# kcroker/Gadget-2.0.7-ngravs

Hardware: AMD Instinct MI355X
Metric: particle-steps/s (tree+PM) (higher is better)
Workload: dtype f64

## Files before the change

gadget-2.0.7-ngravs_amd/csrc/capi.hip:

```cpp
#include "engine.hpp"
#include "../../include/ngravs_peano.h"
#include <chrono>
#include <cmath>

static thread_local std::string g_create_error;

void ngravs_report(ngravs_ctx *ctx, int code, const std::string &msg)
{
  if(ctx)
    ctx->last_error = msg;
  else
    g_create_error = msg;
  if(ctx && ctx->on_fatal)
    ctx->on_fatal(code, msg.c_str());
  else
    fprintf(stderr, "task %d: endrun called with an error level of %d (%s)\n", ctx ? ctx->cfg.rank : 0, code, msg.c_str());
}

__global__ void k_pack_strided_f64(const unsigned char *src, long long stride, int ncomp, long long n, double *dst)
{
  long long i = blockIdx.x * (long long)blockDim.x + threadIdx.x;
  if(i >= n)
    return;
  const double *s = reinterpret_cast<const double *>(src + i * stride);
// ... 942 lines not shown
      return NGRAVS_ERR_NO_DEVICE;
    }
  uint32_t gp[8] = {0}, gw[8] = {0};
  if(hipExtStreamGetCUMask(sp, 8, gp) != hipSuccess || hipExtStreamGetCUMask(sw, 8, gw) != hipSuccess || memcmp(gp, mp, sizeof mp) ||
     memcmp(gw, mw, sizeof mw))
    {
      (void)hipStreamDestroy(sp);
      (void)hipStreamDestroy(sw);
      (void)hipGetLastError();
      return NGRAVS_ERR_NO_DEVICE;
    }
  c->pm_stream = sp;
  c->walk_stream = sw;
  c->pm_stream_cus = R;
  return NGRAVS_OK;
}

static bool overlap_eligible(const ngravs_ctx *c)
{
  return c->cfg.pmgrid && c->cfg.periodic && c->cfg.world_size == 1 && !c->top.on && c->cfg.walk_mode == NGRAVS_WALK_GROUP &&
         c->n > 0 && c->n_local > 0;
}

static int gravity_tree_impl(ngravs_ctx *c, hipEvent_t pm_done)
{
  if(!c || !c->have_order)
    return NGRAVS_ERR_STATE;
  (void)hipSetDevice(c->cfg.device);
  int rc;
  if(!c->have_tree)
    {
      int64_t nn = ngravs_force_treebuild(c);
      if(nn < 0)
        return (int)nn;
    }
  else if(c->tree_stale && (rc = ngravs_force_update_tree(c)))
    return rc;
  if((rc = ensure_table(c)))
    return rc;
  if(c->n_local == 0)
    {
      c->stats.t_treewalk = 0;
      c->stats.walk_kernel_ms = 0;
      c->stats.interactions = 0;
      c->stats.n_active = 0;
      c->have_acc = true;
      return NGRAVS_OK;
    }
  HIP_TRY(c, hipEventRecord(c->ev0, c->stream));
  const bool masked = (pm_done || (c->tune.pm_cus > 0 && overlap_eligible(c))) && masked_streams(c, pm_done ? c->pm_stream_cus : c->tune.pm_cus) == NGRAVS_OK;
  if(masked)
    {
      HIP_TRY(c, hipStreamWaitEvent(c->walk_stream, c->ev0, 0));
      {
        OnStream on(c, c->walk_stream, c->device_cus - c->pm_stream_cus);
        if((rc = walk_run(c)))
          return rc;
      }
      HIP_TRY(c, hipEventRecord(c->ev_walk, c->walk_stream));
      HIP_TRY(c, hipStreamWaitEvent(c->stream, c->ev_walk, 0));
    }
  else if((rc = walk_run(c)))
    return rc;
  if(pm_done)
    HIP_TRY(c, hipStreamWaitEvent(c->stream, pm_done, 0));
  if((rc = walk_finish(c)))
    return rc;
  HIP_TRY(c, hipEventRecord(c->ev1, c->stream));
  c->stats.t_treewalk = ev_ms(c) * 1e-3;
  float kms = 0;
  (void)hipEventSynchronize(c->evk1);
  (void)hipEventElapsedTime(&kms, c->evk0, c->evk1);
  c->stats.walk_kernel_ms = kms;
  double h[2] = {0, 0};
  HIP_TRY(c, hipMemcpyAsync(h, c->red_tmp.p, 2 * sizeof(double), hipMemcpyDeviceToHost, c->stream));
  HIP_TRY(c, hipStreamSynchronize(c->stream));
  c->stats.interactions = h[0];
  c->stats.n_active = (int64_t)h[1];
  c->have_acc = true;
  if(c->cfg.pmgrid && c->cfg.walk_mode == NGRAVS_WALK_GROUP && h[1] > 0 && c->cfg.box_size > 0)
    {
      const double reach = (c->cfg.group_reach > 0 ? c->cfg.group_reach : NGRAVS_GROUP_REACH) * c->asmth;
      const double ntot = c->top.on && c->top.total_count > 0 ? c->top.total_count : (double)c->n;
      const double L = c->cfg.box_size, expect = 4.18879020478639 * reach * reach * reach * ntot / (L * L * L);
      const bool dense = c->walk_ntargets < 0 || c->walk_dense_tlist;
      if(expect > 0 && dense)
        {
          const double f_sg = c->walk_sg >= 4 ? 1.0 : (c->walk_sg >= 2 ? 1857.0 / 1393.0 : 1857.0 / 1079.0);
          const double f_s = c->walk_spread >= 2 ? 1079.0 / 871.0 : 1.0;
          c->walk_ia_ratio = (h[0] / h[1]) / expect * f_sg * f_s;
        }
    }
  if(c->shard_count > 0 && c->extent_override)
    hipLaunchKernelGGL(k_cost_update, GRID1(c->shard_count), 0, c->stream, c->s_idx.p, c->s_active.p, c->r_nint.p,
                       (long long)c->shard_first, (long long)c->shard_count, c->in_cost.p);
  return NGRAVS_OK;
}

extern "C" int ngravs_gravity_tree(ngravs_ctx *c) { return gravity_tree_impl(c, nullptr); }

static int pm_on_masked_stream(ngravs_ctx *c)
{
  HIP_TRY(c, hipEventRecord(c->ev_fork, c->stream));
  HIP_TRY(c, hipStreamWaitEvent(c->pm_stream, c->ev_fork, 0));
  OnStream on(c, c->pm_stream, c->pm_stream_cus);
  HIP_TRY(c, hipEventRecord(c->ev_pm0, c->stream));
  int rc = pm_run(c);
  if(rc)
    return rc;
  HIP_TRY(c, hipEventRecord(c->ev_pm1, c->stream));
  return NGRAVS_OK;
}

extern "C" int ngravs_pmforce_periodic(ngravs_ctx *c)
{
  if(!c || !c->have_particles)
    return NGRAVS_ERR_STATE;
  (void)hipSetDevice(c->cfg.device);
  int rc;
  if(!c->have_order && (rc = ngravs_domain_decomposition(c)))
    return rc;
  if(!c->have_tree)
// ... 45 lines not shown
            c->pm_auto_cus = 8 * m;
          break;
        }
    }
  return c->pm_auto_cus;
}

extern "C" int ngravs_compute_accelerations(ngravs_ctx *c, int pm_step)
{
  if(!c || !c->have_particles)
    return NGRAVS_ERR_STATE;
  int rc;
  if((rc = domain_decomposition_impl(c, !(pm_step && c->cfg.pmgrid))))
    return rc;
  c->last_pm_cus = 0;
  if(!(pm_step && c->cfg.pmgrid))
    return ngravs_gravity_tree(c);
  const int R = choose_pm_cus(c);
  if(R > 0 && masked_streams(c, R) == NGRAVS_OK)
    {
      int64_t nn = ngravs_force_treebuild(c);
      if(nn < 0)
        return (int)nn;
      if((rc = pm_on_masked_stream(c)))
        return rc;
      if((rc = gravity_tree_impl(c, c->ev_pm1)))
        return rc;
      float ms = 0;
      (void)hipEventElapsedTime(&ms, c->ev_pm0, c->ev_pm1);
      c->stats.t_pm = ms * 1e-3;
      c->last_pm_cus = R;
      if(c->tune.pm_cus < 0 && ms > c->stats.walk_kernel_ms)
        c->pm_auto_cus = R < 32 ? R + 8 : 0;
      return NGRAVS_OK;
    }
  if((rc = ngravs_pmforce_periodic(c)))
    return rc;
  if((rc = ngravs_gravity_tree(c)))
    return rc;
  if(overlap_eligible(c) && c->tune.pm_cus < 0 && c->pm_auto_cus < 0)
    {
      c->pm_solo_ms = c->stats.t_pm * 1e3;
      c->walk_solo_ms = c->stats.walk_kernel_ms;
      c->pm_solo_steps++;
    }
  return NGRAVS_OK;
}

static int download_strided(ngravs_ctx *c, const void *dsrc, size_t elem, int ncomp, int64_t n, void *dst, int64_t stride,
// ... 1035 lines not shown
```

gadget-2.0.7-ngravs_amd/csrc/engine.hpp:

```cpp
#pragma once
#include <hip/hip_runtime.h>
#include <cstdint>
#include <cstdio>
#include <cstdlib>
#include <cstring>
#include <string>
#include <vector>
#include "../../include/ngravs_host.h"

#define NG_MAX NGRAVS_MAX_GRAVS
#define NTAB NGRAVS_NTAB
#define TREE_BITS NGRAVS_TREE_BITS
#define FLAG_BUCKET 64
#define FLAG_PSEUDO 128
#define FLAG_PARTIAL 256
#define MAX_LEVELS (TREE_BITS + 1)

struct ngravs_ctx;

#define HIP_TRY(ctx, expr)                                                                        \
  do                                                                                              \
    {                                                                                             \
      hipError_t e__ = (expr);                                                                    \
      if(e__ != hipSuccess)                                                                       \
        {                                                                                         \
          ngravs_report(ctx, NGRAVS_ERR_NO_DEVICE, std::string(#expr) + ": " + hipGetErrorString(e__)); \
          return NGRAVS_ERR_NO_DEVICE;                                                            \
        }                                                                                         \
    }                                                                                             \
  while(0)

void ngravs_report(ngravs_ctx *ctx, int code, const std::string &msg);

template <typename T> struct DevBuf
{
  T *p = nullptr;
  size_t cap = 0;
  int ensure(size_t n)
// ... 231 lines not shown
  long long walk_unopened = 0;
  int walk_unit_state = 4;
  double walk_ia_ratio = 0;
  bool all_active = true;
  DevBuf<int> walk_ovf;
  DevBuf<int> walk_counters;
  DevBuf<double> r_acc, r_pm, r_oldacc;
  DevBuf<int> r_nint;
  int pm_plan_n = 0;
  void *fft_fwd = nullptr, *fft_inv = nullptr;
  DevBuf<double> pm_rho;
  DevBuf<double> pm_force;
  DevBuf<double> pm_phi;
  DevBuf<double> pm_orig;
  DevBuf<double> out_tmp;
  DevBuf<float> out_tmpf;
  std::vector<unsigned char> host_stage;
  ngravs_stats_t stats;
  hipEvent_t ev0 = nullptr, ev1 = nullptr, evk0 = nullptr, evk1 = nullptr;
  std::vector<hipEvent_t> ev_batch;
  int walk_batches = 0;
  int walk_lcap = 0;
  int walk_scap = 0;
  std::string last_error;
  std::vector<ngravs_user_fn_t> user_fns;
  std::vector<ngravs_user_lattice_t> user_lat;
  DevBuf<double> user_tab;
  UserTabs user_ut = {};
  bool user_ready = false;
  double user_soft[NGRAVS_NTYPES] = {0, 0, 0, 0, 0, 0};
  int last_walk_kernel = 0;
  hipStream_t pm_stream = nullptr, walk_stream = nullptr;
  int pm_stream_cus = 0;
  int device_cus = 0;
  int stream_cus = 0;
  int last_pm_cus = 0;
  double pm_solo_ms = 0, walk_solo_ms = 0;
  int pm_solo_steps = 0;
  int pm_auto_cus = -1;
  hipEvent_t ev_fork = nullptr, ev_pm0 = nullptr, ev_pm1 = nullptr, ev_walk = nullptr;
  DevBuf<int> probe_out;
  DevBuf<double> user_green;
  long long user_green_nk2 = 0;
  DevBuf<double> sph_vel_in, sph_h_in;
  DevBuf<double> sph_vel;
  DevBuf<int> sph_tlist;
// ... 64 lines not shown
         (cfg.law_spline[i][j] >= NGRAVS_SPLINE_BAMBAM && cfg.law_spline[i][j] < NGRAVS_SPLINE_USER0))
        return true;
  return false;
}
static inline bool cfg_has_user(const ngravs_config_t &cfg)
{
  for(int i = 0; i < cfg.n_gravs; i++)
    for(int j = 0; j < cfg.n_gravs; j++)
      if(cfg.law_accel[i][j] >= NGRAVS_LAW_USER0 || cfg.law_spline[i][j] >= NGRAVS_SPLINE_USER0)
        return true;
  return false;
}
int user_check_config(const ngravs_config_t *cfg, const ngravs_user_fn_t *fns, int nfns, const ngravs_user_lattice_t *lat, int nlat,
                      std::string &why);
ngravs_lattice_fn user_lattice_fn(const ngravs_ctx *c, int a, int b);
bool user_lattice_complete(const ngravs_ctx *c);
int user_lattice_tabulate(ngravs_lattice_fn fn, double box, double *out, std::string &why);
void ngravs_report(ngravs_ctx *ctx, int code, const std::string &msg);
int user_tables_ensure(ngravs_ctx *c, double r_need);
int user_green_ensure(ngravs_ctx *c);
double user_normed(const ngravs_user_fn_t *fns, int nfns, int law, double k2);
void make_walk_params(const ngravs_ctx *c, WalkParams *wp);
int walk_run(ngravs_ctx *c);
int walk_finish(ngravs_ctx *c);
int direct_run(ngravs_ctx *c, const int *d_idx, int64_t nt, double *d_acc);
int direct_run_targets(ngravs_ctx *c, const double4 *d_tpm, const int *d_ttype, int64_t nt, double *d_acc, double r_need = 0);
int eval_ring_slots(const WalkParams &wp, bool yuk, int waves);
int launch_eval_ring(ngravs_ctx *c, const TreeView &tv, const WalkParams &wp, bool yuk, int nblk, int waves, int K, const int *region,
                     const int *gcount, long long g0, long long nb, int lcap, int scap, int S, const int *tlist, int SG, long long t_count);
#define SPH_KC1 2.546479089470
#define SPH_KC2 15.278874536822
#define SPH_KC3 45.836623610466
#define SPH_KC4 30.557749073644
#define SPH_KC5 5.092958178941
#define SPH_KC6 (-15.278874536822)
#define SPH_NORM_COEFF 4.188790204786
#define SPH_MAXITER 150
__host__ __device__ inline void sph_spline(double u, double hinv3, double hinv4, double *wk, double *dwk)
{
  if(u < 0.5)
    {
      *wk = hinv3 * (SPH_KC1 + SPH_KC2 * (u - 1) * u * u);
      *dwk = hinv4 * u * (SPH_KC3 * u - SPH_KC4);
    }
  else
    {
// ... 53 lines not shown
```

gadget-2.0.7-ngravs_amd/csrc/kernels_tree.hip:

```cpp
#include "engine.hpp"
#include <hipcub/hipcub.hpp>


__device__ __forceinline__ int key_digit(unsigned long long k, int level)
{
  return (int)((k >> (3 * (TREE_BITS - 1 - level))) & 7ull);
}

#define TB 128

__global__ __launch_bounds__(TB) void k_split(const unsigned long long *__restrict__ key, const int *__restrict__ n_first,
                                              const int *__restrict__ n_count, const int *__restrict__ lv, int level,
                                              int *__restrict__ n_child, int *__restrict__ n_nchild, int *__restrict__ blocksum,
                                              const int *__restrict__ n_top = nullptr, const int *__restrict__ t_child = nullptr,
                                              const int *__restrict__ t_gcnt = nullptr)
{
  __shared__ int wsum[TB / 64];
  const int node0 = lv[2 * level], nnodes_level = lv[2 * level + 1];
  const int nvb = (nnodes_level + TB - 1) / TB;
  for(int vb = blockIdx.x; vb < nvb; vb += gridDim.x)
    {
      const int t = vb * TB + threadIdx.x;
      int nn = 0;
      if(t < nnodes_level)
// ... 464 lines not shown
                          const int *__restrict__ n_first, const int *__restrict__ n_count,
                          const int *__restrict__ n_child, const double4 *__restrict__ n_geo,
                          double4 *__restrict__ n_mom, int *__restrict__ n_flags, int node0, int nnodes_level,
                          WalkParams wp, double4 *__restrict__ geo_rw = nullptr, int *__restrict__ n_npart = nullptr,
                          int *__restrict__ n_count_rw = nullptr)
{
  int t = blockIdx.x * blockDim.x + threadIdx.x;
  if(t >= nnodes_level)
    return;
  int node = node0 + t;
  double m[NG], sx[NG], sy[NG], sz[NG];
  int np[NG];
#pragma unroll
  for(int g = 0; g < NG; g++)
    {
      m[g] = sx[g] = sy[g] = sz[g] = 0;
      np[g] = 0;
    }
  SoftAcc sa;
  sa.maxsofttype = 7;
  sa.diff = 0;
  int cnt_acc = 0;
  int fl = n_flags[node];
  const double4 geo0 = n_geo[node];
  double need = 0;
  auto add_particle_v = [&](const double4 v, const int ty) {
    if(geo_rw)
      need = fmax(need, fmax(fabs(v.x - geo0.x), fmax(fabs(v.y - geo0.y), fabs(v.z - geo0.z))));
    int gg = wp.t2g[ty];
#pragma unroll
    for(int g = 0; g < NG; g++)
      if(g == gg)
        {
          np[g]++;
          m[g] += v.w;
          sx[g] += v.w * v.x;
          sy[g] += v.w * v.y;
          sz[g] += v.w * v.z;
        }
    soft_merge(sa, ty, 0, wp.fsoft);
    cnt_acc++;
  };
  auto add_particle = [&](int p) {
    double4 v = s_pm[p];
    if(geo_rw)
      need = fmax(need, fmax(fabs(v.x - geo0.x), fmax(fabs(v.y - geo0.y), fabs(v.z - geo0.z))));
    int ty = s_type[p];
    int gg = wp.t2g[ty];
#pragma unroll
    for(int g = 0; g < NG; g++)
      if(g == gg)
        {
          np[g]++;
          m[g] += v.w;
          sx[g] += v.w * v.x;
          sy[g] += v.w * v.y;
          sz[g] += v.w * v.z;
        }
    soft_merge(sa, ty, 0, wp.fsoft);
    cnt_acc++;
  };
  if(fl & FLAG_BUCKET)
    {
      int f = n_first[node], cnt = n_count[node];
      for(int p = f; p < f + cnt; p++)
        add_particle(p);
    }
  else
    {
      const int4 *cp = reinterpret_cast<const int4 *>(n_child + 8 * (long long)node);
      const int4 c_lo = cp[0], c_hi = cp[1];
      const int ch[8] = {c_lo.x, c_lo.y, c_lo.z, c_lo.w, c_hi.x, c_hi.y, c_hi.z, c_hi.w};
      constexpr int B = NG == 1 ? 4 : 2;
#pragma unroll
      for(int k0 = 0; k0 < 8; k0 += B)
        {
          double4 rec[B][NG];
          int aux[B], cnt_c[B];
#pragma unroll
          for(int q = 0; q < B; q++)
            {
              const int c = ch[k0 + q];
              aux[q] = 0;
              cnt_c[q] = 0;
              if(c <= -2)
                {
                  rec[q][0] = s_pm[-2 - c];
                  aux[q] = s_type[-2 - c];
                }
              else if(c >= 0)
                {
#pragma unroll
                  for(int g = 0; g < NG; g++)
                    rec[q][g] = n_mom[(long long)c * NG + g];
                  aux[q] = n_flags[c];
                  if(n_count_rw)
                    cnt_c[q] = n_count_rw[c];
                }
            }
#pragma unroll
          for(int q = 0; q < B; q++)
            {
              const int c = ch[k0 + q];
              if(c == -1)
                continue;
              if(c <= -2)
                add_particle_v(rec[q][0], aux[q]);
              else
                {
#pragma unroll
                  for(int g = 0; g < NG; g++)
                    {
                      const double4 cm = rec[q][g];
                      if(n_npart)
                        np[g] += n_npart[(long long)c * NG + g];
                      m[g] += cm.w;
                      sx[g] += cm.w * cm.x;
                      sy[g] += cm.w * cm.y;
                      sz[g] += cm.w * cm.z;
                    }
                  const int cf = aux[q];
                  soft_merge(sa, (cf >> 2) & 7, (cf >> 5) & 1, wp.fsoft);
                  cnt_acc += cnt_c[q];
                  if(geo_rw)
                    {
                      const double4 cg = n_geo[c];
                      need = fmax(need, fmax(fabs(cg.x - geo0.x), fmax(fabs(cg.y - geo0.y), fabs(cg.z - geo0.z))) + 0.5 * cg.w);
                    }
                }
            }
        }
    }
  double4 geo = geo0;
  if(geo_rw && 2.0 * need > geo.w)
    {
      geo.w = 2.0 * need;
      geo_rw[node] = geo;
    }
#pragma unroll
  for(int g = 0; g < NG; g++)
    {
      double4 o;
      if(m[g] > 0)
        {
          o.x = sx[g] / m[g];
          o.y = sy[g] / m[g];
          o.z = sz[g] / m[g];
        }
      else
        {
          o.x = geo.x;
          o.y = geo.y;
          o.z = geo.z;
        }
      o.w = m[g];
      n_mom[(long long)node * NG + g] = o;
      if(n_npart)
        n_npart[(long long)node * NG + g] = np[g];
    }
  n_flags[node] = (fl & (FLAG_BUCKET | FLAG_PSEUDO | FLAG_PARTIAL)) | (4 * sa.maxsofttype + 32 * sa.diff);
  if(n_count_rw && !(fl & FLAG_BUCKET))
    n_count_rw[node] = cnt_acc;
}

template <int NG>
__global__ void k_top_moments(const int *__restrict__ n_top, const int *__restrict__ t_child, const double *__restrict__ gsum,
                              const double4 *__restrict__ n_geo, double4 *__restrict__ n_mom, int *__restrict__ n_flags, int node0,
                              int nnodes_level, WalkParams wp)
{
  int t = blockIdx.x * blockDim.x + threadIdx.x;
  if(t >= nnodes_level)
    return;
  const int node = node0 + t, fl = n_flags[node], tn = n_top[node];
  if(tn < 0 || (t_child[tn] < 0 && !(fl & FLAG_PSEUDO)))
    return;
  const double *s = gsum + (size_t)tn * TOP_CW(NG);
  const double4 geo = n_geo[node];
#pragma unroll
  for(int g = 0; g < NG; g++)
    {
      double4 o;
      const double m = s[7 + 4 * g];
      if(m > 0)
        {
          o.x = s[7 + 4 * g + 1] / m;
          o.y = s[7 + 4 * g + 2] / m;
          o.z = s[7 + 4 * g + 3] / m;
        }
      else
        {
          o.x = geo.x;
          o.y = geo.y;
          o.z = geo.z;
        }
      o.w = m;
      n_mom[(long long)node * NG + g] = o;
    }
  SoftAcc sa;
  sa.maxsofttype = 7;
  sa.diff = 0;
  for(int ty = 0; ty < NGRAVS_NTYPES; ty++)
    if(s[1 + ty] > 0)
      soft_merge(sa, ty, 0, wp.fsoft);
  n_flags[node] = (fl & (FLAG_BUCKET | FLAG_PSEUDO | FLAG_PARTIAL)) | (4 * sa.maxsofttype + 32 * sa.diff);
}

static int tree_top_moments(ngravs_ctx *c)
{
  const TopTree &t = c->top;
  WalkParams wp;
  make_walk_params(c, &wp);
  for(int l = (t.h.depth < c->nlevels - 1 ? t.h.depth : c->nlevels - 1); l >= 0; l--)
    {
      const long long l0 = c->level_start[l], lc = c->level_start[l + 1] - l0;
      if(lc <= 0)
        continue;
      const unsigned nb = (unsigned)((lc + 127) / 128);
      switch(c->cfg.n_gravs)
        {
        case 1:
          hipLaunchKernelGGL(k_top_moments<1>, dim3(nb), dim3(128), 0, c->stream, c->n_top.p, t.child.p, t.gsum.p, c->n_geo.p, c->n_mom.p,
                             c->n_flags.p, (int)l0, (int)lc, wp);
          break;
        case 2:
          hipLaunchKernelGGL(k_top_moments<2>, dim3(nb), dim3(128), 0, c->stream, c->n_top.p, t.child.p, t.gsum.p, c->n_geo.p, c->n_mom.p,
                             c->n_flags.p, (int)l0, (int)lc, wp);
          break;
// ... 254 lines not shown
```

gadget-2.0.7-ngravs_amd/csrc/kernels_walk.hip:

```cpp
#include "engine.hpp"
#include "walk_device.hpp"
#include "eval_asm.inc"
#include <hipcub/hipcub.hpp>
#include <type_traits>

__device__ __forceinline__ double bam_eta(int law, double target, double m, double N, double eps)
{
  if(law == NGRAVS_LAW_BAMBAM)
    return 4.0 * M_PI * eps / (target + m / N);
  if(law == NGRAVS_LAW_SOURCEBAM)
    return 4.0 * M_PI * eps * N / m;
  return 4.0 * M_PI * eps / target;
}
__device__ __forceinline__ double bam_accel(int law, double target, double m, double r, double N, double eps)
{
  double eta = bam_eta(law, target, m, N, eps), rho = 2 * target * m / M_PI;
  double reta = r * eta, reta2 = reta * reta, eta3 = eta * eta * eta;
  if(reta < 0.1)
    return rho * eta3 * (2.0 * r / 3.0 - 4.0 * reta2 * r / 5.0 + 6.0 * reta2 * reta2 * r / 7.0);
  return rho * eta3 * (atan(reta) / (reta2 * eta) - 1.0 / (reta * eta * (1 + reta2)));
}
__device__ __forceinline__ double bam_spline(int law, double target, double m, double r, double N, double eps)
{
  double eta = bam_eta(law, target, m, N, eps), rho = 2 * target * m / M_PI;
// ... 502 lines not shown
          }
        const bool wave_open = __any(open ? 1 : 0) != 0;
        if(wave_open && takes_part && !open)
          lane_skip = sp + 1;
        return wave_open;
      };
      dfs(lat_visit, lat_particle);
    }
  if(valid)
    {
      r_acc[3 * ti + 0] = ax;
      r_acc[3 * ti + 1] = ay;
      r_acc[3 * ti + 2] = az;
      r_nint[ti] = nint;
    }
}

#pragma clang fp contract(fast)

#define GW_MAXWAVES 12
#define GW_STACK 8192
#define GW2_WAVE_LDS (sizeof(double4) + (sizeof(double4) + 4 * sizeof(float) + 1) * 128)
#define GW_NLEAF 8

#define GW2_ITEMS 16384

#define GW3_LIST_MIN 4096
#define GW3_LIST_MAX 65536
#define GW3_STK_MIN 4096
#define GW3_STK_MAX 65536
#define GW2_MAXWAVES 16
#define GW3_TBLOCK 256
#define GW3_RING 1024

template <int NG, bool PM, bool YUK, bool TAB_LDS, bool LATT, int MODE, bool USR = false>
__global__ __launch_bounds__(MODE == 1 ? GW3_TBLOCK : (MODE == 2 ? GW2_MAXWAVES : GW_MAXWAVES) * 64) void k_walk_group2(
    TreeView tv, const double4 *__restrict__ s_pm, const unsigned char *__restrict__ s_type,
    const double *__restrict__ s_oldacc, const unsigned char *__restrict__ s_active,
    const double *__restrict__ table, WalkParams wp, long long t_first, long long t_count, int *__restrict__ counter,
    int *__restrict__ stack_base, int *__restrict__ err_flag, double *__restrict__ r_acc, int *__restrict__ r_nint,
    int *__restrict__ region_base, int *__restrict__ gcount, long long g_first, long long g_cnt, int lcap, int scap,
    int *__restrict__ glist, int S, int G0, const int *__restrict__ tlist, int SG)
{
  constexpr int ES = 1;
  extern __shared__ __attribute__((aligned(16))) unsigned char smem[];
  __shared__ int ring_s[MODE == 1 ? (GW3_TBLOCK / 64) * GW3_RING : 1];
// ... 873 lines not shown
            if constexpr(MODE == 1)
              {
                if(full)
                  {
                    overflow = true;
                    break;
                  }
              }
            else if(full)
              phase2_all();
          }
          const int nb = sp < WAVE ? sp : WAVE;
          sp -= nb;
          st_nodes += nb;
          st_batches++;
          int my = -1;
          if(MODE == 1 && sp >= ring_lo)
            my = lane < nb ? ring[(sp + lane) & (GW3_RING - 1)] : -1;
          else
            my = lane < nb ? STK(sp + lane) : -1;
          wave_sync();
          int dec = 0;
          int first = 0, count = 0;
          unsigned massmask = 0;
          bool pseudo_hit = false;
          int4 ch_lo = {-1, -1, -1, -1}, ch_hi = {-1, -1, -1, -1};
          if(my >= 0)
            {
              const double4 geo = tv.geo[my];
              const int fl = tv.flags[my];
              const double len = geo.w, half = 0.5 * len;
              double cx = geo.x - bcx, cy = geo.y - bcy, cz = geo.z - bcz;
              double wx = cx, wy = cy, wz = cz;
              if(!nowrap)
                {
                  wx = nearest_abs(cx, wp.box, invbox);
                  wy = nearest_abs(cy, wp.box, invbox);
                  wz = nearest_abs(cz, wp.box, invbox);
                }
              const int mst = (fl >> 2) & 7;
              bool drop = (mst == 7);
              if(PM && !drop)
                {
                  double q0 = fmax(0.0, fabs(wx) - bhx - half), q1 = fmax(0.0, fabs(wy) - bhy - half),
                         q2 = fmax(0.0, fabs(wz) - bhz - half);
                  if(q0 * q0 + q1 * q1 + q2 * q2 >= wp.reach2)
                    drop = true;
                }
              if(!drop)
                {
                  first = tv.first[my];
                  count = tv.count[my];
                  double r2min = BIG, r2far = 0, summass = 0;
#pragma unroll
                  for(int g = 0; g < NG; g++)
                    {
                      const double4 mom = tv.mom[(long long)my * NG + g];
                      summass += mom.w;
                      massmask |= (mom.w != 0.0) ? (1u << g) : 0u;
                      double dx = mom.x - bcx, dy = mom.y - bcy, dz = mom.z - bcz;
                      if(!nowrap)
                        {
                          dx = nearest_abs(dx, wp.box, invbox);
                          dy = nearest_abs(dy, wp.box, invbox);
                          dz = nearest_abs(dz, wp.box, invbox);
                        }
                      double a0 = fmax(0.0, fabs(dx) - bhx), a1 = fmax(0.0, fabs(dy) - bhy), a2 = fmax(0.0, fabs(dz) - bhz);
                      double r2g = a0 * a0 + a1 * a1 + a2 * a2;
                      r2min = r2g < r2min ? r2g : r2min;
                      r2far = r2g > r2far ? r2g : r2far;
                    }
                  if(PM && r2min > wp.rcut2)
                    {
                      double eff = wp.rcut + half;
                      if(fabs(wx) - bhx > eff || fabs(wy) - bhy > eff || fabs(wz) - bhz > eff)
// ... 3 lines not shown
                    {
                      bool open;
                      if(wp.use_theta)
                        open = len * len > r2min * wp.theta2;
                      else
                        {
                          open = summass * len * len > r2min * r2min * aold_min;
                          if(!open)
                            open = (fabs(cx) - bhx < 0.60 * len) && (fabs(cy) - bhy < 0.60 * len) &&
                                   (fabs(cz) - bhz < 0.60 * len);
                        }
                      const double hs_node = usoft ? wp.fsoft[0] : wp.fsoft[mst];
                      if(!open && hT_min < hs_node && r2far < hs_node * hs_node && ((fl >> 5) & 1))
                        open = true;
                      if(open && (fl & FLAG_PSEUDO))
                        {
                          open = false;
                          pseudo_hit = true;
                        }
                      if(open)
                        dec = ((fl & FLAG_BUCKET) || (count <= wp.nleaf && !(fl & FLAG_PARTIAL))) ? 3 : 2;
                      else
                        dec = 1;
                    }
                }
            }
          {
            const unsigned long long ph_ = __ballot(pseudo_hit ? 1 : 0);
            if(ph_ != 0ull && lane == 0)
              atomicAdd(&counter[4], __popcll(ph_));
          }
          if(dec == 2)
            {
              const int4 *cp = reinterpret_cast<const int4 *>(tv.child + 8 * (long long)my);
              ch_lo = cp[0];
              ch_hi = cp[1];
            }
#pragma unroll
          for(int g = 0; g < NG; g++)
            {
              const bool pg = dec == 1 && ((massmask >> g) & 1u);
              unsigned long long mask = __ballot(pg ? 1 : 0);
              if(pg)
                lists[g][n_items[g] + lane_prefix(mask)] = -1 - (my * NG + g);
              n_items[g] += __popcll(mask);
            }
          const int chv[8] = {ch_lo.x, ch_lo.y, ch_lo.z, ch_lo.w, ch_hi.x, ch_hi.y, ch_hi.z, ch_hi.w};
          unsigned sp8 = 0;
          if(NG > 1)
            {
              unsigned char ty8[8];
#pragma unroll
              for(int q = 0; q < 8; q++)
                {
                  int pi = 0;
                  if(dec == 2 && chv[q] <= -2)
                    pi = -2 - chv[q];
                  if(dec == 3 && q < count)
                    pi = first + q;
                  ty8[q] = s_type[pi];
                }
#pragma unroll
              for(int q = 0; q < 8; q++)
                sp8 |= ((wp.t2g_packed >> (2 * ty8[q])) & 3u) << (2 * q);
            }
          if(__any(dec >= 2))
            {
              int itemv[8];
              unsigned cnt_pack = 0;
              unsigned cnt_g2 = 0;
#pragma unroll
              for(int q = 0; q < 8; q++)
                {
                  int it = -1;
                  if(dec == 2)
                    it = chv[q];
                  else if(dec == 3 && q < count)
                    it = -2 - (first + q);
                  itemv[q] = it;
                  const int sgq = (int)((sp8 >> (2 * q)) & 3u);
                  const bool isp = it <= -2;
                  cnt_pack += it >= 0 ? 1u : (isp && sgq < 2 ? (1u << 10) << (10 * sgq) : 0u);
                  cnt_g2 += isp && sgq == 2 ? 1u : 0u;
                }
              unsigned inc = cnt_pack, inc2 = cnt_g2;
#pragma unroll
              for(int off = 1; off < WAVE; off <<= 1)
// ... 586 lines not shown
    return c->stream_cus;
  hipDeviceProp_t prop;
  if(hipGetDeviceProperties(&prop, c->cfg.device) == hipSuccess && prop.multiProcessorCount > 0)
    return prop.multiProcessorCount;
  return 256;
}

struct EvalLds
{
  int waves;
  size_t bytes;
};
static EvalLds eval_lds(const WalkParams &wp, bool tables, int max_waves)
{
  const size_t fixed = (tables ? sizeof(double) * (wp.ntab_lds + wp.exp_tab) * NTAB : 0) + 40 * sizeof(double);
  int waves = (int)((160 * 1024 - fixed) / GW2_WAVE_LDS);
  if(waves > max_waves)
    waves = max_waves;
  if(waves < 1)
    waves = 1;
  return {waves, fixed + (size_t)waves * GW2_WAVE_LDS};
}

template <int NG, int PM, int YUK, int TAB_LDS, int LATT, int USR>
static int launch_group2_t(Row<NG, PM, YUK, TAB_LDS, LATT, USR>, ngravs_ctx *c, const WalkParams &wp, int *glist, int nlist)
{
  const int S0 = c->walk_spread > 1 ? c->walk_spread : 1, G0 = (WAVE / S0) * (glist ? c->walk_sg : 1);
  int S = S0;
  if(glist)
    {
      const int want = nlist <= 4096 ? 64 : (nlist <= 65536 ? 8 : 1);
      S = want > S0 ? want : S0;
    }
  const int G = WAVE / S;
  const int ncu = walk_cus(c);
  const EvalLds l = eval_lds(wp, PM && TAB_LDS, GW_MAXWAVES);
  const int waves = l.waves;
  const size_t lds = l.bytes;
  long long ngroups = glist ? (long long)nlist * (G0 / G) : (walk_tcount(c) + G - 1) / G;
  long long nblk = ncu;
  if(nblk > (ngroups + waves - 1) / waves)
    nblk = (ngroups + waves - 1) / waves;
  if(nblk < 1)
    nblk = 1;
  if(c->walk_stack.ensure((size_t)nblk * waves * (GW_STACK + (size_t)NG * GW2_ITEMS)) || c->walk_counters.ensure(32))
    return NGRAVS_ERR_NOMEM;
  if(glist)
    HIP_TRY(c, hipMemsetAsync(c->walk_counters.p + 8, 0, sizeof(int) * 8, c->stream));
  else
    HIP_TRY(c, hipMemsetAsync(c->walk_counters.p, 0, sizeof(int) * 32, c->stream));
  auto kern = k_walk_group2<NG, PM, YUK, TAB_LDS, LATT, 0, USR>;
  HIP_TRY(c, hipFuncSetAttribute(reinterpret_cast<const void *>(kern), hipFuncAttributeMaxDynamicSharedMemorySize, (int)lds));
  hipLaunchKernelGGL(kern, dim3((unsigned)nblk), dim3(waves * 64), lds, c->stream, tree_view(c), c->s_pm.p,
                     c->s_type.p, c->s_oldacc.p, c->s_active.p, LATT ? c->lat.p : c->table.p, wp, (long long)c->shard_first,
                     walk_tcount(c), c->walk_counters.p, c->walk_stack.p, c->walk_counters.p + 1, c->r_acc.p,
                     c->r_nint.p, (int *)nullptr, (int *)nullptr, 0ll, glist ? (long long)nlist : 0ll, 0, 0, glist, S, G0, walk_tlist(c), 1);
  return NGRAVS_OK;
}

static int walk_unit_next(int st, double r)
{
  if(!(r > 0))
    return st;
  if(st == 4)
    return r > 2.0 ? 1 : (r > 1.4 ? 2 : 4);
  if(st == 2)
    return r > 2.0 ? 1 : (r < 1.2 ? 4 : 2);
  return r < 1.2 ? 4 : (r < 1.7 ? 2 : 1);
}

template <int NG, int PM, int YUK, int TAB_LDS, int LATT, int USR>
static int launch_group3_t(Row<NG, PM, YUK, TAB_LDS, LATT, USR>, ngravs_ctx *c, const WalkParams &wp)
{
  const int ncu = walk_cus(c);
  const int max_waves = c->tune.walk_waves > 0 && c->tune.walk_waves < GW2_MAXWAVES ? c->tune.walk_waves : GW2_MAXWAVES;
// ... 4 lines not shown
  const long long ngroups = (walk_tcount(c) + G - 1) / G;
  int SG = (PM && (c->walk_ntargets < 0 || c->walk_dense_tlist)) ? 4 : 1;
  if(SG == 4)
    SG = c->walk_unit_state = walk_unit_next(c->walk_unit_state, c->walk_ia_ratio);
  if(c->tune.walk_sg >= 1)
    SG = c->tune.walk_sg;
  if(SG != c->walk_sg)
    c->walk_lcap = 0;
  c->walk_sg = SG;
  const long long nunits = (ngroups + SG - 1) / SG;
  if(c->walk_lcap < 1024)
    {
      c->walk_lcap = (NG == 1 ? 2 : 1) * (SG > 1 ? 2 : 1) * GW3_LIST_MIN;
      if(c->tune.walk_lcap >= 1024)
        c->walk_lcap = c->tune.walk_lcap;
    }
  if(c->walk_scap < GW3_STK_MIN)
    c->walk_scap = GW3_STK_MIN;
  c->walk_lcap &= ~3;
  const int lcap = c->walk_lcap, scap = c->walk_scap;
  const size_t region_ints = (size_t)NG * lcap + scap;
  long long batch = 1 << 20;
  size_t cap_bytes = (size_t)8 << 30;
  {
    size_t free_b = 0, total_b = 0;
    if(hipMemGetInfo(&free_b, &total_b) == hipSuccess)
      {
        free_b += c->walk_stack.cap * sizeof(int);
        if(free_b / 4 > cap_bytes)
          cap_bytes = free_b / 4;
        if(cap_bytes > ((size_t)64 << 30))
          cap_bytes = (size_t)64 << 30;
      }
  }
  if(c->tune.walk_batch > 0)
    {
      batch = c->tune.walk_batch;
      cap_bytes = (size_t)64 << 30;
    }
  while(batch > 8192 && (size_t)batch * region_ints * sizeof(int) > cap_bytes)
    batch /= 2;
  if(batch > nunits)
    batch = nunits;
  if(batch < 1)
    batch = 1;
  if(c->walk_stack.ensure((size_t)batch * (region_ints + NG + 2)) || c->walk_counters.ensure(32) ||
     c->walk_ovf.ensure((size_t)nunits))
    return NGRAVS_ERR_NOMEM;
  int *region = c->walk_stack.p, *gcount = c->walk_stack.p + (size_t)batch * region_ints;
  HIP_TRY(c, hipMemsetAsync(c->walk_counters.p, 0, sizeof(int) * 32, c->stream));
  auto kt = k_walk_group2<NG, PM, YUK, TAB_LDS, LATT, 1, USR>;
  auto ke = k_walk_group2<NG, PM, YUK, TAB_LDS, LATT, 2, USR>;
  HIP_TRY(c, hipFuncSetAttribute(reinterpret_cast<const void *>(ke), hipFuncAttributeMaxDynamicSharedMemorySize, (int)lds));
  int ringK = 0, ring_waves = waves;
  if constexpr(PM && TAB_LDS && !LATT && !USR)
    if(c->tune.walk_ring)
      {
        ring_waves = max_waves;
        ringK = eval_ring_slots(wp, YUK, ring_waves);
        if(c->tune.walk_ring_k >= 4 && c->tune.walk_ring_k < ringK)
          ringK = c->tune.walk_ring_k;
        if(ringK)
          waves = ring_waves;
      }
  const size_t nbatches = (size_t)((nunits + batch - 1) / batch);
  while(c->ev_batch.size() < 3 * nbatches)
    {
      hipEvent_t e;
      HIP_TRY(c, hipEventCreate(&e));
      c->ev_batch.push_back(e);
    }
  c->walk_batches = (int)nbatches;
  size_t ib = 0;
  for(long long u0 = 0; u0 < nunits; u0 += batch, ib++)
    {
      const long long nbu = nunits - u0 < batch ? nunits - u0 : batch;
// ... 86 lines not shown
      return cbrt(vol_per_target * 64.0) > 2.5 * sqrt(wp.reach2) ? 64 : 0;
    }
  if(tuned > 1)
    return tuned;
  if(tuned == 0)
    {
      const long long g64 = (walk_tcount(c) + WAVE - 1) / WAVE;
      if(pm && c->walk_unit_state == 1 && c->walk_ia_ratio > 2.0)
        return 2;
      if(!pm && !latt && g64 > 0 && g64 < 2048)
        return g64 < 1024 ? 4 : 2;
    }
  return 0;
}

static int walk_read_back(ngravs_ctx *c, int *flag, unsigned long long (&st64)[4])
{
  HIP_TRY(c, hipMemcpyAsync(flag, c->walk_counters.p + 1, sizeof(int), hipMemcpyDeviceToHost, c->stream));
  HIP_TRY(c, hipMemcpyAsync(st64, c->walk_counters.p + 16, 4 * sizeof(unsigned long long), hipMemcpyDeviceToHost, c->stream));
  HIP_TRY(c, hipStreamSynchronize(c->stream));
  return NGRAVS_OK;
}

int walk_run(ngravs_ctx *c)
{
  const long long n = c->n;
  if(c->r_acc.ensure(3 * n) || c->r_nint.ensure(n) || c->r_oldacc.ensure(n))
    return NGRAVS_ERR_NOMEM;
  const bool latt = c->cfg.periodic && !c->cfg.pmgrid;
  if(latt)
    {
      int rcl = ensure_lattice(c);
      if(rcl)
        return rcl;
    }
  {
    int rcu = user_tables_ensure(c, latt ? lattice_reach(c) : user_reach(c));
    if(rcu)
      return rcu;
  }
  WalkParams wp;
  make_walk_params(c, &wp);
  LawIds li;
  make_law_ids(c, &li);
  c->walk_ntargets = -1;
  const bool strict = c->cfg.walk_mode == NGRAVS_WALK_STRICT;
  if(c->top.on && c->cfg.pmgrid)
// ... 22 lines not shown
    }
  const bool pm = c->cfg.pmgrid != 0;
  HIP_TRY(c, hipEventRecord(c->evk0, c->stream));
  int rc = NGRAVS_OK;
  bool used_split = false;
  if(strict)
    {
      if(c->walk_counters.ensure(32))
        return NGRAVS_ERR_NOMEM;
      HIP_TRY(c, hipMemsetAsync(c->walk_counters.p, 0, sizeof(int) * 32, c->stream));
      c->last_walk_kernel = wp.user ? NGRAVS_KERNEL_STRICT_USER : NGRAVS_KERNEL_STRICT;
      const int key[] = {c->cfg.n_gravs, pm, latt, wp.user != 0};
      rc = dispatch(c, StrictRows{}, key, [&](auto row) { return launch_strict(row, c, wp, li); });
    }
  else
    {
      c->walk_spread = walk_spread_choice(c, wp, latt);
      rc = launch_group(c, wp, &used_split);
    }
  if(rc != NGRAVS_OK)
    return rc;
  HIP_TRY(c, hipEventRecord(c->evk1, c->stream));
  HIP_TRY(c, hipGetLastError());
  c->walk_unopened = 0;
  if(strict && c->top.on)
    {
      int flag = 0;
      HIP_TRY(c, hipMemcpyAsync(&flag, c->walk_counters.p + 1, sizeof(int), hipMemcpyDeviceToHost, c->stream));
      HIP_TRY(c, hipStreamSynchronize(c->stream));
      if(flag & 4)
        {
          ngravs_report(c, NGRAVS_ERR_STATE, "the walk opens a top-tree leaf whose particles were not imported: the opening criterion or OldAcc "
                                             "changed since the decomposition (decompose again before this walk)");
          return NGRAVS_ERR_STATE;
        }
    }
  if(!strict)
    {
      int flag = 0;
      unsigned long long st64[4] = {0, 0, 0, 0};
      if((rc = walk_read_back(c, &flag, st64)))
        return rc;
      if(used_split)
        {
          int ovf[2] = {0, 0};
          HIP_TRY(c, hipMemcpy(ovf, c->walk_counters.p + 2, 2 * sizeof(int), hipMemcpyDeviceToHost));
// ... 27 lines not shown
      for(int b = 0; b < c->walk_batches; b++)
        {
          float te = 0, tt = 0;
          (void)hipEventElapsedTime(&tt, c->ev_batch[3 * b], c->ev_batch[3 * b + 1]);
          (void)hipEventElapsedTime(&te, c->ev_batch[3 * b + 1], c->ev_batch[3 * b + 2]);
          c->stats.reserved[4] += te;
          c->stats.reserved[6] += tt;
        }
      c->stats.reserved[5] = c->walk_batches;
      {
        int unop = 0;
        HIP_TRY(c, hipMemcpy(&unop, c->walk_counters.p + 4, sizeof(int), hipMemcpyDeviceToHost));
        c->walk_unopened = unop;
      }
      if(flag)
        {
          ngravs_report(c, NGRAVS_ERR_TREE, "group walk: pending-node LIFO overflow");
          return NGRAVS_ERR_TREE;
        }
    }
  return NGRAVS_OK;
}

int walk_finish(ngravs_ctx *c)
{
  const int bs = 256;
  unsigned nb = (unsigned)((c->shard_count + bs - 1) / bs);
  nb = nb > 4096u ? 4096u : nb;
  if(c->red_tmp.ensure(2))
    return NGRAVS_ERR_NOMEM;
  HIP_TRY(c, hipMemsetAsync(c->red_tmp.p, 0, 2 * sizeof(double), c->stream));
  if(nb == 0)
    return NGRAVS_OK;
  hipLaunchKernelGGL(k_finish, dim3(nb), dim3(bs), 0, c->stream, (long long)c->shard_first, (long long)c->shard_count,
                     c->s_active.p, c->r_acc.p, c->r_pm.p, c->r_oldacc.p, c->cfg.G, (c->have_pm && c->cfg.pmgrid) ? 1 : 0,
                     c->r_nint.p, c->red_tmp.p);
  HIP_TRY(c, hipGetLastError());
  return NGRAVS_OK;
}

using DirectRows = Table<Row<0>, Row<1>>;
template <int USER> static auto direct_kernel(Row<USER>) { return k_direct<USER>; }
static int direct_launch(ngravs_ctx *c, double r_need, const int *d_idx, int64_t nt, double *d_acc, const double4 *d_tpm, const int *d_ttype)
{
  if(c->cfg.periodic && !user_lattice_complete(c))
    {
// ... 34 lines not shown
```

Before: 625.4 million.

## Enqueue walk before PM, precompute species codes in node flags, cache launch setup

```diff
diff --git a/gadget-2.0.7-ngravs_amd/csrc/capi.hip b/gadget-2.0.7-ngravs_amd/csrc/capi.hip
--- a/gadget-2.0.7-ngravs_amd/csrc/capi.hip
+++ b/gadget-2.0.7-ngravs_amd/csrc/capi.hip
@@ -988,8 +988,9 @@
          c->n > 0 && c->n_local > 0;
 }
 
-static int gravity_tree_impl(ngravs_ctx *c, hipEvent_t pm_done)
-{
+static int gravity_tree_begin(ngravs_ctx *c, bool beside_pm, bool *masked, bool *empty)
+{
+  *masked = *empty = false;
   if(!c || !c->have_order)
     return NGRAVS_ERR_STATE;
   (void)hipSetDevice(c->cfg.device);
@@ -1011,22 +1012,34 @@
       c->stats.interactions = 0;
       c->stats.n_active = 0;
       c->have_acc = true;
+      *empty = true;
       return NGRAVS_OK;
     }
   HIP_TRY(c, hipEventRecord(c->ev0, c->stream));
-  const bool masked = (pm_done || (c->tune.pm_cus > 0 && overlap_eligible(c))) && masked_streams(c, pm_done ? c->pm_stream_cus : c->tune.pm_cus) == NGRAVS_OK;
+  *masked = (beside_pm || (c->tune.pm_cus > 0 && overlap_eligible(c))) && masked_streams(c, beside_pm ? c->pm_stream_cus : c->tune.pm_cus) == NGRAVS_OK;
+  if(*masked)
+    {
+      HIP_TRY(c, hipStreamWaitEvent(c->walk_stream, c->ev0, 0));
+      OnStream on(c, c->walk_stream, c->device_cus - c->pm_stream_cus);
+      return walk_enqueue(c);
+    }
+  return walk_enqueue(c);
+}
+
+static int gravity_tree_end(ngravs_ctx *c, bool masked, hipEvent_t pm_done)
+{
+  int rc;
   if(masked)
     {
-      HIP_TRY(c, hipStreamWaitEvent(c->walk_stream, c->ev0, 0));
       {
         OnStream on(c, c->walk_stream, c->device_cus - c->pm_stream_cus);
-        if((rc = walk_run(c)))
+        if((rc = walk_complete(c)))
           return rc;
       }
       HIP_TRY(c, hipEventRecord(c->ev_walk, c->walk_stream));
       HIP_TRY(c, hipStreamWaitEvent(c->stream, c->ev_walk, 0));
     }
-  else if((rc = walk_run(c)))
+  else if((rc = walk_complete(c)))
     return rc;
   if(pm_done)
     HIP_TRY(c, hipStreamWaitEvent(c->stream, pm_done, 0));
@@ -1063,7 +1076,12 @@
   return NGRAVS_OK;
 }
 
-extern "C" int ngravs_gravity_tree(ngravs_ctx *c) { return gravity_tree_impl(c, nullptr); }
+extern "C" int ngravs_gravity_tree(ngravs_ctx *c)
+{
+  bool masked, empty;
+  const int rc = gravity_tree_begin(c, false, &masked, &empty);
+  return (rc || empty) ? rc : gravity_tree_end(c, masked, nullptr);
+}
 
 static int pm_on_masked_stream(ngravs_ctx *c)
 {
@@ -1155,9 +1173,12 @@
       int64_t nn = ngravs_force_treebuild(c);
       if(nn < 0)
         return (int)nn;
+      bool masked, empty;
+      if((rc = gravity_tree_begin(c, true, &masked, &empty)))
+        return rc;
       if((rc = pm_on_masked_stream(c)))
         return rc;
-      if((rc = gravity_tree_impl(c, c->ev_pm1)))
+      if(!empty && (rc = gravity_tree_end(c, masked, c->ev_pm1)))
         return rc;
       float ms = 0;
       (void)hipEventElapsedTime(&ms, c->ev_pm0, c->ev_pm1);
diff --git a/gadget-2.0.7-ngravs_amd/csrc/engine.hpp b/gadget-2.0.7-ngravs_amd/csrc/engine.hpp
--- a/gadget-2.0.7-ngravs_amd/csrc/engine.hpp
+++ b/gadget-2.0.7-ngravs_amd/csrc/engine.hpp
@@ -5,6 +5,7 @@
 #include <cstdlib>
 #include <cstring>
 #include <string>
+#include <utility>
 #include <vector>
 #include "../../include/ngravs_host.h"
 
@@ -14,6 +15,9 @@
 #define FLAG_BUCKET 64
 #define FLAG_PSEUDO 128
 #define FLAG_PARTIAL 256
+#define FLAG_SPECIES_SHIFT 9
+#define FLAG_SPECIES_SLOTS 8
+#define FLAG_SPECIES_MASK (0xffff << FLAG_SPECIES_SHIFT)
 #define MAX_LEVELS (TREE_BITS + 1)
 
 struct ngravs_ctx;
@@ -291,6 +295,11 @@
   int walk_batches = 0;
   int walk_lcap = 0;
   int walk_scap = 0;
+  bool walk_used_split = false;
+  long long walk_cap_n = -1;
+  size_t walk_cap_stack = 0;
+  size_t walk_cap_bytes = 0;
+  std::vector<std::pair<const void *, size_t>> walk_lds_set;
   std::string last_error;
   std::vector<ngravs_user_fn_t> user_fns;
   std::vector<ngravs_user_lattice_t> user_lat;
@@ -401,6 +410,8 @@
 double user_normed(const ngravs_user_fn_t *fns, int nfns, int law, double k2);
 void make_walk_params(const ngravs_ctx *c, WalkParams *wp);
 int walk_run(ngravs_ctx *c);
+int walk_enqueue(ngravs_ctx *c);
+int walk_complete(ngravs_ctx *c);
 int walk_finish(ngravs_ctx *c);
 int direct_run(ngravs_ctx *c, const int *d_idx, int64_t nt, double *d_acc);
 int direct_run_targets(ngravs_ctx *c, const double4 *d_tpm, const int *d_ttype, int64_t nt, double *d_acc, double r_need = 0);
diff --git a/gadget-2.0.7-ngravs_amd/csrc/kernels_tree.hip b/gadget-2.0.7-ngravs_amd/csrc/kernels_tree.hip
--- a/gadget-2.0.7-ngravs_amd/csrc/kernels_tree.hip
+++ b/gadget-2.0.7-ngravs_amd/csrc/kernels_tree.hip
@@ -510,6 +510,8 @@
   sa.diff = 0;
   int cnt_acc = 0;
   int fl = n_flags[node];
+  unsigned sp_slot = 0, sp_range = 0;
+  auto species = [&](const int ty) { return (wp.t2g_packed >> (2 * ty)) & 3u; };
   const double4 geo0 = n_geo[node];
   double need = 0;
   auto add_particle_v = [&](const double4 v, const int ty) {
@@ -529,7 +531,7 @@
     soft_merge(sa, ty, 0, wp.fsoft);
     cnt_acc++;
   };
-  auto add_particle = [&](int p) {
+  auto add_particle = [&](int p) -> int {
     double4 v = s_pm[p];
     if(geo_rw)
       need = fmax(need, fmax(fabs(v.x - geo0.x), fmax(fabs(v.y - geo0.y), fabs(v.z - geo0.z))));
@@ -547,12 +549,17 @@
         }
     soft_merge(sa, ty, 0, wp.fsoft);
     cnt_acc++;
+    return ty;
   };
   if(fl & FLAG_BUCKET)
     {
       int f = n_first[node], cnt = n_count[node];
       for(int p = f; p < f + cnt; p++)
-        add_particle(p);
+        {
+          const int ty = add_particle(p);
+          if(NG > 1 && p - f < FLAG_SPECIES_SLOTS)
+            sp_range |= species(ty) << (2 * (p - f));
+        }
     }
   else
     {
@@ -582,8 +589,7 @@
                   for(int g = 0; g < NG; g++)
                     rec[q][g] = n_mom[(long long)c * NG + g];
                   aux[q] = n_flags[c];
-                  if(n_count_rw)
-                    cnt_c[q] = n_count_rw[c];
+                  cnt_c[q] = n_count[c];
                 }
             }
 #pragma unroll
@@ -593,7 +599,16 @@
               if(c == -1)
                 continue;
               if(c <= -2)
-                add_particle_v(rec[q][0], aux[q]);
+                {
+                  if(NG > 1)
+                    {
+                      const unsigned sg = species(aux[q]);
+                      sp_slot |= sg << (2 * (k0 + q));
+                      if(cnt_acc < FLAG_SPECIES_SLOTS)
+                        sp_range |= sg << (2 * cnt_acc);
+                    }
+                  add_particle_v(rec[q][0], aux[q]);
+                }
               else
                 {
 #pragma unroll
@@ -609,6 +624,8 @@
                     }
                   const int cf = aux[q];
                   soft_merge(sa, (cf >> 2) & 7, (cf >> 5) & 1, wp.fsoft);
+                  if(NG > 1 && cnt_acc < FLAG_SPECIES_SLOTS)
+                    sp_range |= (((unsigned)cf >> FLAG_SPECIES_SHIFT) & 0xffffu) << (2 * cnt_acc);
                   cnt_acc += cnt_c[q];
                   if(geo_rw)
                     {
@@ -646,7 +663,10 @@
       if(n_npart)
         n_npart[(long long)node * NG + g] = np[g];
     }
-  n_flags[node] = (fl & (FLAG_BUCKET | FLAG_PSEUDO | FLAG_PARTIAL)) | (4 * sa.maxsofttype + 32 * sa.diff);
+  const int cnt_node = (n_count_rw && !(fl & FLAG_BUCKET)) ? cnt_acc : n_count[node];
+  const bool range_coded = (fl & FLAG_BUCKET) || (cnt_node <= FLAG_SPECIES_SLOTS && !(fl & FLAG_PARTIAL));
+  const unsigned sp = NG > 1 ? ((range_coded ? sp_range : sp_slot) & 0xffffu) : 0u;
+  n_flags[node] = (fl & (FLAG_BUCKET | FLAG_PSEUDO | FLAG_PARTIAL)) | (4 * sa.maxsofttype + 32 * sa.diff) | (int)(sp << FLAG_SPECIES_SHIFT);
   if(n_count_rw && !(fl & FLAG_BUCKET))
     n_count_rw[node] = cnt_acc;
 }
@@ -690,7 +710,7 @@
   for(int ty = 0; ty < NGRAVS_NTYPES; ty++)
     if(s[1 + ty] > 0)
       soft_merge(sa, ty, 0, wp.fsoft);
-  n_flags[node] = (fl & (FLAG_BUCKET | FLAG_PSEUDO | FLAG_PARTIAL)) | (4 * sa.maxsofttype + 32 * sa.diff);
+  n_flags[node] = (fl & (FLAG_BUCKET | FLAG_PSEUDO | FLAG_PARTIAL | FLAG_SPECIES_MASK)) | (4 * sa.maxsofttype + 32 * sa.diff);
 }
 
 static int tree_top_moments(ngravs_ctx *c)
diff --git a/gadget-2.0.7-ngravs_amd/csrc/kernels_walk.hip b/gadget-2.0.7-ngravs_amd/csrc/kernels_walk.hip
--- a/gadget-2.0.7-ngravs_amd/csrc/kernels_walk.hip
+++ b/gadget-2.0.7-ngravs_amd/csrc/kernels_walk.hip
@@ -548,6 +548,7 @@
 #define GW_STACK 8192
 #define GW2_WAVE_LDS (sizeof(double4) + (sizeof(double4) + 4 * sizeof(float) + 1) * 128)
 #define GW_NLEAF 8
+static_assert(GW_NLEAF <= FLAG_SPECIES_SLOTS, "a node handed over as a leaf must be range-coded (k_moments)");
 
 #define GW2_ITEMS 16384
 
@@ -1467,7 +1468,7 @@
           wave_sync();
           int dec = 0;
           int first = 0, count = 0;
-          unsigned massmask = 0;
+          unsigned info = 0;
           bool pseudo_hit = false;
           int4 ch_lo = {-1, -1, -1, -1}, ch_hi = {-1, -1, -1, -1};
           if(my >= 0)
@@ -1496,6 +1497,7 @@
                 {
                   first = tv.first[my];
                   count = tv.count[my];
+                  unsigned massmask = 0;
                   double r2min = BIG, r2far = 0, summass = 0;
 #pragma unroll
                   for(int g = 0; g < NG; g++)
@@ -1545,6 +1547,8 @@
                         dec = ((fl & FLAG_BUCKET) || (count <= wp.nleaf && !(fl & FLAG_PARTIAL))) ? 3 : 2;
                       else
                         dec = 1;
+                      static_assert(FLAG_PARTIAL << 1 == 1 << FLAG_SPECIES_SHIFT, "one shift takes both out of the flags word");
+                      info = open ? (NG > 1 ? ((unsigned)fl >> (FLAG_SPECIES_SHIFT - 1)) & 0x1ffffu : 0u) : massmask;
                     }
                 }
             }
@@ -1562,30 +1566,25 @@
 #pragma unroll
           for(int g = 0; g < NG; g++)
             {
-              const bool pg = dec == 1 && ((massmask >> g) & 1u);
+              const bool pg = dec == 1 && ((info >> g) & 1u);
               unsigned long long mask = __ballot(pg ? 1 : 0);
               if(pg)
                 lists[g][n_items[g] + lane_prefix(mask)] = -1 - (my * NG + g);
               n_items[g] += __popcll(mask);
             }
           const int chv[8] = {ch_lo.x, ch_lo.y, ch_lo.z, ch_lo.w, ch_hi.x, ch_hi.y, ch_hi.z, ch_hi.w};
-          unsigned sp8 = 0;
+          unsigned sp8 = NG > 1 ? info >> 1 : 0u;
           if(NG > 1)
             {
-              unsigned char ty8[8];
-#pragma unroll
-              for(int q = 0; q < 8; q++)
+              const bool remap = dec == 2 && count <= FLAG_SPECIES_SLOTS && !(info & 1u);
+              if(__any(remap))
                 {
-                  int pi = 0;
-                  if(dec == 2 && chv[q] <= -2)
-                    pi = -2 - chv[q];
-                  if(dec == 3 && q < count)
-                    pi = first + q;
-                  ty8[q] = s_type[pi];
+                  unsigned r = 0;
+#pragma unroll
+                  for(int q = 0; q < 8; q++)
+                    r |= ((sp8 >> (2 * ((-2 - chv[q] - first) & 7))) & 3u) << (2 * q);
+                  sp8 = remap ? r : sp8;
                 }
-#pragma unroll
-              for(int q = 0; q < 8; q++)
-                sp8 |= ((wp.t2g_packed >> (2 * ty8[q])) & 3u) << (2 * q);
             }
           if(__any(dec >= 2))
             {
@@ -2218,6 +2217,22 @@
   return {waves, fixed + (size_t)waves * GW2_WAVE_LDS};
 }
 
+static int walk_dyn_lds(ngravs_ctx *c, const void *kern, size_t lds)
+{
+  for(auto &e : c->walk_lds_set)
+    if(e.first == kern)
+      {
+        if(e.second == lds)
+          return NGRAVS_OK;
+        HIP_TRY(c, hipFuncSetAttribute(kern, hipFuncAttributeMaxDynamicSharedMemorySize, (int)lds));
+        e.second = lds;
+        return NGRAVS_OK;
+      }
+  HIP_TRY(c, hipFuncSetAttribute(kern, hipFuncAttributeMaxDynamicSharedMemorySize, (int)lds));
+  c->walk_lds_set.emplace_back(kern, lds);
+  return NGRAVS_OK;
+}
+
 template <int NG, int PM, int YUK, int TAB_LDS, int LATT, int USR>
 static int launch_group2_t(Row<NG, PM, YUK, TAB_LDS, LATT, USR>, ngravs_ctx *c, const WalkParams &wp, int *glist, int nlist)
 {
@@ -2246,7 +2261,8 @@
   else
     HIP_TRY(c, hipMemsetAsync(c->walk_counters.p, 0, sizeof(int) * 32, c->stream));
   auto kern = k_walk_group2<NG, PM, YUK, TAB_LDS, LATT, 0, USR>;
-  HIP_TRY(c, hipFuncSetAttribute(reinterpret_cast<const void *>(kern), hipFuncAttributeMaxDynamicSharedMemorySize, (int)lds));
+  if(int rl = walk_dyn_lds(c, reinterpret_cast<const void *>(kern), lds))
+    return rl;
   hipLaunchKernelGGL(kern, dim3((unsigned)nblk), dim3(waves * 64), lds, c->stream, tree_view(c), c->s_pm.p,
                      c->s_type.p, c->s_oldacc.p, c->s_active.p, LATT ? c->lat.p : c->table.p, wp, (long long)c->shard_first,
                      walk_tcount(c), c->walk_counters.p, c->walk_stack.p, c->walk_counters.p + 1, c->r_acc.p,
@@ -2297,17 +2313,23 @@
   const size_t region_ints = (size_t)NG * lcap + scap;
   long long batch = 1 << 20;
   size_t cap_bytes = (size_t)8 << 30;
-  {
-    size_t free_b = 0, total_b = 0;
-    if(hipMemGetInfo(&free_b, &total_b) == hipSuccess)
-      {
-        free_b += c->walk_stack.cap * sizeof(int);
-        if(free_b / 4 > cap_bytes)
-          cap_bytes = free_b / 4;
-        if(cap_bytes > ((size_t)64 << 30))
-          cap_bytes = (size_t)64 << 30;
-      }
-  }
+  if(c->walk_cap_n == c->n && c->walk_cap_stack == c->walk_stack.cap && c->walk_cap_bytes > 0)
+    cap_bytes = c->walk_cap_bytes;
+  else
+    {
+      size_t free_b = 0, total_b = 0;
+      if(hipMemGetInfo(&free_b, &total_b) == hipSuccess)
+        {
+          free_b += c->walk_stack.cap * sizeof(int);
+          if(free_b / 4 > cap_bytes)
+            cap_bytes = free_b / 4;
+          if(cap_bytes > ((size_t)64 << 30))
+            cap_bytes = (size_t)64 << 30;
+          c->walk_cap_n = c->n;
+          c->walk_cap_stack = c->walk_stack.cap;
+          c->walk_cap_bytes = cap_bytes;
+        }
+    }
   if(c->tune.walk_batch > 0)
     {
       batch = c->tune.walk_batch;
@@ -2326,7 +2348,8 @@
   HIP_TRY(c, hipMemsetAsync(c->walk_counters.p, 0, sizeof(int) * 32, c->stream));
   auto kt = k_walk_group2<NG, PM, YUK, TAB_LDS, LATT, 1, USR>;
   auto ke = k_walk_group2<NG, PM, YUK, TAB_LDS, LATT, 2, USR>;
-  HIP_TRY(c, hipFuncSetAttribute(reinterpret_cast<const void *>(ke), hipFuncAttributeMaxDynamicSharedMemorySize, (int)lds));
+  if(int rl = walk_dyn_lds(c, reinterpret_cast<const void *>(ke), lds))
+    return rl;
   int ringK = 0, ring_waves = waves;
   if constexpr(PM && TAB_LDS && !LATT && !USR)
     if(c->tune.walk_ring)
@@ -2459,7 +2482,7 @@
   return NGRAVS_OK;
 }
 
-int walk_run(ngravs_ctx *c)
+int walk_enqueue(ngravs_ctx *c)
 {
   const long long n = c->n;
   if(c->r_acc.ensure(3 * n) || c->r_nint.ensure(n) || c->r_oldacc.ensure(n))
@@ -2528,6 +2551,17 @@
     return rc;
   HIP_TRY(c, hipEventRecord(c->evk1, c->stream));
   HIP_TRY(c, hipGetLastError());
+  c->walk_used_split = used_split;
+  return NGRAVS_OK;
+}
+
+int walk_complete(ngravs_ctx *c)
+{
+  const bool strict = c->cfg.walk_mode == NGRAVS_WALK_STRICT;
+  const bool used_split = c->walk_used_split;
+  int rc = NGRAVS_OK;
+  WalkParams wp;
+  make_walk_params(c, &wp);
   c->walk_unopened = 0;
   if(strict && c->top.on)
     {
@@ -2601,6 +2635,12 @@
   return NGRAVS_OK;
 }
 
+int walk_run(ngravs_ctx *c)
+{
+  const int rc = walk_enqueue(c);
+  return rc ? rc : walk_complete(c);
+}
+
 int walk_finish(ngravs_ctx *c)
 {
   const int bs = 256;
```

Result: faster. 634.2 million (median of 6 runs) (+1.4%).
